# modelscope/dash-infer

Hardware: NVIDIA H100
Metric: decode tokens/sec/GPU Qwen2-7B int4-IQ b=1..64; HBM GB/s vs roofline (higher is better)
Workload: dtype bf16 activations x int4 weights (fp32 accumulate), none KV

## Files before the change

### dash-infer_b200/csrc/wq_gemm.cu

```cuda
#include <cstdio>
#include <cstdlib>
#include <cstring>
#include <map>
#include <mutex>
#include <new>

#include "b2_common.cuh"
#include "comm_shared.cuh"
#include "wq_gemm_shared.cuh"

namespace b2 {

constexpr int kWarps = 8;
constexpr int kThreads = kWarps * 32 + 32;
constexpr int kStageBytes = 8192;
static_assert(kBN == kWarps * 16, "one n16 tile per consumer warp");

struct GemmParams {
  const uint8_t* packed;
  const float2* sz;
  const __nv_bfloat16* A;
  int64_t lda;
  __nv_bfloat16* C;
  int64_t ldc;
// ... 736 lines not shown
    const __nv_bfloat16* sc = (pair && r >= 64) ? scales2 : scales;
    const __nv_bfloat16* zr = (pair && r >= 64) ? zeros2 : zeros;
    float2 v = make_float2(0.f, 0.f);
    if (n < N) {
      const __nv_bfloat16 sv = sc[(int64_t)gi * N + n], zv = zr[(int64_t)gi * N + n];
      v = fp16 ? make_float2(Ft<true>::to_f(sv), Ft<true>::to_f(zv) + zbias) : make_float2(Ft<false>::to_f(sv), Ft<false>::to_f(zv) + zbias);
    }
    dst[i] = v;
  }
}

}

using namespace b2;

struct Plan {
  bool valid = false;
  int S = 1, xt = 1, smem = 0, quanta = 1, nst_log2 = 2;
  bool cluster = false;
};

struct b2_gemm_wq {
  b2_gemm_wq_desc d;
  int Kp = 0, Np = 0, KT = 0, NG = 0, G = 1, group_tiles = 0;
  int group_k = 0;
  size_t tile_bytes = 0, packed_bytes = 0;
  void* packed = nullptr;
  bool own_packed = false;
  float2* sz = nullptr;
  bool own_sz = false;
  unsigned* counters = nullptr;
  Plan plans[2];
  int tc_S = 0;
  int tc_S2 = 0;
  bool pair = false;
  int device = 0;
};

typedef void (*gemm_kernel_t)(const GemmParams);

template <int WBITS, bool GROUPED, bool H>
static gemm_kernel_t pick_mt(int mt) {
  switch (mt) {
    case 1: return wq_gemm_kernel<WBITS, 1, GROUPED, H>;
    default: return wq_gemm_kernel<WBITS, 2, GROUPED, H>;
  }
}
template <bool H>
static gemm_kernel_t pick_kernel_ft(int wbits, bool grouped, int mt) {
  if (wbits == 4) return grouped ? pick_mt<4, true, H>(mt) : pick_mt<4, false, H>(mt);
  if (wbits == 8) return grouped ? pick_mt<8, true, H>(mt) : pick_mt<8, false, H>(mt);
  return pick_mt<16, false, H>(mt);
}
static gemm_kernel_t pick_kernel(int wbits, bool grouped, int mt, bool fp16) {
  return fp16 ? pick_kernel_ft<true>(wbits, grouped, mt) : pick_kernel_ft<false>(wbits, grouped, mt);
}
static int stage_bytes_of(int wbits) { return wbits == 16 ? WTraits<16>::STAGE_BYTES : kStageBytes; }
static int tile_bytes_of(int wbits) { return wbits == 4 ? WTraits<4>::TILE_BYTES : (wbits == 8 ? WTraits<8>::TILE_BYTES : WTraits<16>::TILE_BYTES); }

static int env_int(const char* name, int dflt) {
  const char* v = getenv(name);
  return v ? atoi(v) : dflt;
}

cudaError_t b2::raise_smem_limit(const void* kern, int smem) {
  static std::mutex mu;
  static std::map<const void*, int> limit;
// ... 209 lines not shown
int b2_gemm_wq_attach_packed(b2_gemm_wq_t h, const void* packed, const void* scales_f32, const void* zeros_f32) {
  (void)zeros_f32;
  if (!h || !packed) return B2_ERR_PARAM;
  if (h->own_packed && h->packed) cudaFree(h->packed);
  h->packed = const_cast<void*>(packed);
  h->own_packed = false;
  if (scales_f32) {
    if (h->own_sz && h->sz) cudaFree(h->sz);
    h->sz = (float2*)const_cast<void*>(scales_f32);
    h->own_sz = false;
  }
  return B2_OK;
}

static int mt_index_for(int M) { return M <= 8 ? 0 : 1; }

constexpr int kTcMinM = 17;

static bool use_tc(const b2_gemm_wq* h, int M) {
  if (h->group_k > 0) return true;
  return M >= kTcMinM && (h->group_tiles == 0 || h->d.wbits == 4);
}

static int make_tc_plan(b2_gemm_wq* h) {
  if (h->tc_S > 0) return B2_OK;
  const int ctas = env_int("B2_GEMM_TC_CTAS_PER_SM", 1);
  auto split_for = [&](int slots, int smax) {
    int S = slots / h->NG;
    if (S > h->KT / 4) S = h->KT / 4;
    if (S > smax) S = smax;
    return S < 1 ? 1 : S;
  };
  h->tc_S = split_for(ctas * sm_count(), env_int("B2_GEMM_TC_MAX_SPLIT", 6));
  h->tc_S2 = split_for(env_int("B2_GEMM_TC_DUAL_SLOTS", 2) * sm_count(), env_int("B2_GEMM_TC_MAX_SPLIT2", 8));
  return B2_OK;
}

static bool tc_dual(const b2_gemm_wq* h) {
  static const int on = env_int("B2_GEMM_TC_DUAL", 1);
  if (!on || h->d.wbits != 4) return false;
  return on >= 2 || h->NG >= 2 * sm_count();
}

size_t b2_gemm_wq_workspace_bytes(b2_gemm_wq_t h, int M) {
  if (!h || M <= 0) return 0;
  if (use_tc(h, M)) {
    if (make_tc_plan(h) != B2_OK) return 0;
    const int sm = h->tc_S > h->tc_S2 ? h->tc_S : h->tc_S2;
    return sm <= 1 ? 16 : (size_t)h->NG * sm * kTcMaxM * kBN * sizeof(float) + 16;
  }
  const int mc = M > kGemvMaxM ? kGemvMaxM : M;
  const int mti = mt_index_for(mc);
  if (make_plan(h, mti) != B2_OK) return 0;
  const Plan& pl = h->plans[mti];
  if (pl.S <= 1 || pl.cluster) return 16;
  return (size_t)h->NG * pl.S * (8 << mti) * (kBN + 1) * sizeof(float) + 16;
}

size_t b2_gemm_wq_algo_bytes(b2_gemm_wq_t h, int M) {
  if (!h) return 0;
  const b2_gemm_wq_desc& d = h->d;
  const size_t mul = h->pair ? 2 : 1;
  size_t w = mul * (size_t)d.K * d.N * d.wbits / 8;
  size_t prm = d.wbits == 16 ? 0 : mul * (size_t)2 * 2 * h->G * d.N;
  return w + prm + (size_t)2 * M * ((size_t)d.K + d.N);
}

int b2_gemm_wq_sumsq_parts(b2_gemm_wq_t h) { return h ? h->NG : 0; }

int b2_gemm_wq_run(b2_gemm_wq_t h, const void* A, int64_t lda, void* C, int64_t ldc, int M, const void* bias,
                   const void* residual, int activation, float alpha, void* workspace, size_t workspace_bytes,
                   void* stream_) {
  return b2_gemm_wq_run_fused(h, A, lda, C, ldc, M, bias, residual, activation, alpha, workspace, workspace_bytes, nullptr, stream_);
}

extern "C" const void* b2_comm_device_view(b2_comm_t c);

static int run_impl(b2_gemm_wq_t h, const void* A, int64_t lda, void* C, int64_t ldc, int M, const void* bias,
                    const void* residual, int activation, float alpha, void* workspace, size_t workspace_bytes,
                    const b2_gemm_fuse* fuse, const CommDev* comm, void* stream_);

int b2_gemm_wq_run_fused(b2_gemm_wq_t h, const void* A, int64_t lda, void* C, int64_t ldc, int M, const void* bias,
// ... 55 lines not shown
                    const b2_gemm_fuse* fuse, const CommDev* comm, void* stream_) {
  if (!h || !A || !C || M <= 0) return B2_ERR_PARAM;
  const bool norm_self = fuse && !fuse->norm_sumsq && fuse->norm_gamma;
  const bool fused = fuse && (fuse->norm_sumsq || fuse->sumsq_out || norm_self || fuse->xg_out);
  if (fused && use_tc(h, M) && !comm) {
    const bool cons = fuse->norm_sumsq != nullptr, prod = fuse->xg_out != nullptr;
    if (norm_self || (cons && fuse->norm_gamma) || (fuse->sumsq_out && !prod)) return B2_ERR_UNSUPPORTED;
    if (cons && (fuse->norm_parts <= 0 || fuse->norm_hidden <= 0)) return B2_ERR_PARAM;
    if (prod) {
      if (!fuse->sumsq_out || !fuse->gamma_out || h->pair || activation != B2_ACT_NONE) return B2_ERR_PARAM;
      if ((h->d.N & 3) || (ldc & 3) || (fuse->ldxg & 3) || (reinterpret_cast<uintptr_t>(C) & 7) ||
          (reinterpret_cast<uintptr_t>(fuse->xg_out) & 7) || (reinterpret_cast<uintptr_t>(fuse->gamma_out) & 7) ||
          (residual && (reinterpret_cast<uintptr_t>(residual) & 7)) || (bias && (reinterpret_cast<uintptr_t>(bias) & 7)))
        return B2_ERR_UNSUPPORTED;
    }
  } else {
    if (norm_self && (fuse->norm_hidden != h->d.K || comm)) return B2_ERR_PARAM;
    if (norm_self && (reinterpret_cast<uintptr_t>(fuse->norm_gamma) & 15)) return B2_ERR_UNSUPPORTED;
    if (fused && (M > 16 || (h->pair && fuse->sumsq_out) || fuse->xg_out)) return B2_ERR_UNSUPPORTED;
    if (fuse && fuse->norm_sumsq && (!fuse->norm_gamma || fuse->norm_parts <= 0 || fuse->norm_hidden <= 0)) return B2_ERR_PARAM;
  }
  if (!h->packed) return B2_ERR_RUNTIME;
  if (M > h->d.max_m) return B2_ERR_LIMIT;
  if (h->group_k > 0 && comm) return B2_ERR_UNSUPPORTED;
  if (h->pair != (activation == B2_ACT_SWIGLU)) return B2_ERR_PARAM;
  if (activation != B2_ACT_SWIGLU && (activation < 0 || activation > B2_ACT_SIGMOID)) return B2_ERR_PARAM;
  if (h->pair && (bias || residual)) return B2_ERR_UNSUPPORTED;
  if ((reinterpret_cast<uintptr_t>(A) & 15) || (lda % 8) != 0) return B2_ERR_UNSUPPORTED;
  if (workspace_bytes < b2_gemm_wq_workspace_bytes(h, M)) return B2_ERR_PARAM;
  cudaStream_t stream = (cudaStream_t)stream_;
  const bool grouped = h->group_tiles > 0;
  if (use_tc(h, M) && !comm) {
    if (int st = make_tc_plan(h)) return st;
    const bool dual = tc_dual(h);
    const int tcs = dual ? h->tc_S2 : h->tc_S;
    if (tcs > 1 && !workspace) return B2_ERR_PARAM;
    for (int m0 = 0; m0 < M; m0 += kTcMaxM) {
      TcLaunch a;
      a.dual = dual;
      a.fp16 = h->d.ft == B2_DT_F16;
      a.packed = (const uint8_t*)h->packed; a.sz = h->sz;
      a.A = (const __nv_bfloat16*)A + (int64_t)m0 * lda; a.lda = lda;
      a.C = (__nv_bfloat16*)C + (int64_t)m0 * ldc; a.ldc = ldc;
      a.bias = (const __nv_bfloat16*)bias;
      a.residual = residual ? (const __nv_bfloat16*)residual + (int64_t)m0 * ldc : nullptr;
      a.ws = (float*)workspace; a.counters = h->counters;
      a.M = (M - m0) > kTcMaxM ? kTcMaxM : (M - m0);
      a.N = h->d.N; a.K = h->d.K; a.Np = h->Np; a.KT = h->KT; a.NG = h->NG; a.S = tcs;
      a.act = activation; a.alpha = alpha;
      a.group_tiles = h->group_tiles;
      a.group_k = h->group_k; a.ngroups = h->G;
      if (fused) {
        a.norm_ld = M;
        if (fuse->norm_sumsq) {
          a.norm_sumsq = fuse->norm_sumsq + m0; a.norm_parts = fuse->norm_parts;
          a.norm_inv_hidden = 1.0f / (float)fuse->norm_hidden; a.norm_eps = fuse->norm_eps;
        }
        if (fuse->xg_out) {
          a.sumsq_out = fuse->sumsq_out + m0;
          a.xg_out = (__nv_bfloat16*)fuse->xg_out + (int64_t)m0 * fuse->ldxg;
          a.gamma_out = (const __nv_bfloat16*)fuse->gamma_out; a.ldxg = fuse->ldxg;
        }
      }
      cudaError_t e = tc_launch(h->d.wbits, a, stream);
      if (e != cudaSuccess) {
        set_last_error("wq_gemm_tc launch", e);
        return B2_ERR_CUDA;
      }
    }
    return B2_OK;
  }
  if (h->d.wbits == 16 && M <= kGemvMaxM && !fused && !comm && h->d.ft == B2_DT_BF16) {
// ... 66 lines not shown
```

### dash-infer_b200/csrc/wq_gemm_shared.cuh

```cuda
#pragma once
#include <cuda.h>

#include "b2_common.cuh"

namespace b2 {

constexpr int kBN = 128;
constexpr int kBK = 64;
constexpr uint32_t kMask4 = 0x00780078u;
constexpr uint32_t kMagic = 0x41804180u;
constexpr uint32_t kMagicHi = 0x43804380u;

__host__ __device__ __forceinline__ int tile_swz(int wbits, int c) {
  return wbits == 4 ? 4 * (c & 1) : (wbits == 8 ? 2 * (c & 3) : 2 * ((c >> 1) & 3));
}

struct TcLaunch {
  const uint8_t* packed;
  const float2* sz;
  const __nv_bfloat16* A;
  int64_t lda;
  __nv_bfloat16* C;
  int64_t ldc;
  const __nv_bfloat16* bias;
  const __nv_bfloat16* residual;
  float* ws;
  unsigned* counters;
  int M, N, K, Np, KT, NG, S;
  int act;
  float alpha;
  const float* a_scale = nullptr;
  const float* tile_sums = nullptr;
  int group_tiles = 0;
  int group_k = 0, ngroups = 1;
  bool fp16 = false;
  bool dual = false;
  const float* norm_sumsq = nullptr;
  int norm_parts = 0, norm_ld = 0;
  float norm_inv_hidden = 0.f, norm_eps = 0.f;
  float* sumsq_out = nullptr;
  __nv_bfloat16* xg_out = nullptr;
  const __nv_bfloat16* gamma_out = nullptr;
  int64_t ldxg = 0;
};
struct Gemv2Launch {
  const uint8_t* packed;
  const __nv_bfloat16* A;
  int64_t lda;
  __nv_bfloat16* C;
  int64_t ldc;
  const __nv_bfloat16* bias;
  const __nv_bfloat16* residual;
  int M, N, K, KT, NG;
  bool pair;
  int act;
  float alpha;
};
struct Gemv2Plan {
  int cb_log2, xt, nst_log2, mt, grid, smem;
};
bool gemv2_plan(const Gemv2Launch& a, Gemv2Plan* plan);
cudaError_t gemv2_launch(const Gemv2Launch& a, const Gemv2Plan& plan, cudaStream_t stream);

constexpr int kGemvMaxM = 16;
constexpr int kTcMaxM = 64;
int tc_smem_bytes(int wbits, bool dual);
cudaError_t tc_launch(int wbits, const TcLaunch& a, cudaStream_t stream);

cudaError_t raise_smem_limit(const void* kern, int smem);

typedef CUresult (*EncodeTiledFn)(CUtensorMap*, CUtensorMapDataType, cuuint32_t, void*, const cuuint64_t*, const cuuint64_t*,
                                  const cuuint32_t*, const cuuint32_t*, CUtensorMapInterleave, CUtensorMapSwizzle,
                                  CUtensorMapL2promotion, CUtensorMapFloatOOBfill);
EncodeTiledFn encode_tiled();

}
```

### dash-infer_b200/csrc/wq_gemm_tc.cu

```cuda
#include <cstdlib>

#include "b2_common.cuh"
#include "wq_gemm_shared.cuh"

namespace b2 {

constexpr int kTcThreads = 384;
constexpr int kTcNM = 64;
constexpr int kTcNSW = 6;
constexpr int kTcNSX = 3;
constexpr int kTcXTile = kTcNM * 128;

__device__ __forceinline__ void wg_fence() { asm volatile("wgmma.fence.sync.aligned;" ::: "memory"); }
__device__ __forceinline__ void wg_commit() { asm volatile("wgmma.commit_group.sync.aligned;" ::: "memory"); }
template <int N>
__device__ __forceinline__ void wg_wait() { asm volatile("wgmma.wait_group.sync.aligned %0;" ::"n"(N) : "memory"); }
__device__ __forceinline__ void wg_fence_acc(float (&d)[32]) {
#pragma unroll
  for (int i = 0; i < 32; ++i) asm volatile("" : "+f"(d[i])::"memory");
}
__device__ __forceinline__ uint64_t wg_desc(uint32_t saddr) {
  return (uint64_t)((saddr >> 4) & 0x3FFF) | ((uint64_t)1 << 16) | ((uint64_t)(1024 >> 4) << 32) | ((uint64_t)1 << 62);
}

#define B2_WG_D16 "{%0,%1,%2,%3,%4,%5,%6,%7,%8,%9,%10,%11,%12,%13,%14,%15}"
#define B2_WG_D32                                                                                                          \
  "{%0,%1,%2,%3,%4,%5,%6,%7,%8,%9,%10,%11,%12,%13,%14,%15,%16,%17,%18,%19,%20,%21,%22,%23,%24,%25,%26,%27,%28,%29,%30,%31}"
#define B2_WG_ACC16(d)                                                                                                       \
  "+f"(d[0]), "+f"(d[1]), "+f"(d[2]), "+f"(d[3]), "+f"(d[4]), "+f"(d[5]), "+f"(d[6]), "+f"(d[7]), "+f"(d[8]), "+f"(d[9]), \
      "+f"(d[10]), "+f"(d[11]), "+f"(d[12]), "+f"(d[13]), "+f"(d[14]), "+f"(d[15])
#define B2_WG_ACC32(d)                                                                                                       \
  B2_WG_ACC16(d), "+f"(d[16]), "+f"(d[17]), "+f"(d[18]), "+f"(d[19]), "+f"(d[20]), "+f"(d[21]), "+f"(d[22]), "+f"(d[23]), \
      "+f"(d[24]), "+f"(d[25]), "+f"(d[26]), "+f"(d[27]), "+f"(d[28]), "+f"(d[29]), "+f"(d[30]), "+f"(d[31])

template <int KIND>
__device__ __forceinline__ void wg_mma(float (&d)[32], const uint32_t (&a)[4], uint64_t desc, bool n32) {
  if (n32) {
    if (KIND == 0)
      asm volatile("{\n\t.reg .pred p;\n\tsetp.ne.b32 p, %21, 0;\n\t"
                   "wgmma.mma_async.sync.aligned.m64n32k16.f32.bf16.bf16 " B2_WG_D16 ", {%16,%17,%18,%19}, %20, p, 1, 1, 0;\n\t}"
                   : B2_WG_ACC16(d) : "r"(a[0]), "r"(a[1]), "r"(a[2]), "r"(a[3]), "l"(desc), "r"(1));
    else if (KIND == 1)
      asm volatile("{\n\t.reg .pred p;\n\tsetp.ne.b32 p, %21, 0;\n\t"
                   "wgmma.mma_async.sync.aligned.m64n32k16.f32.f16.f16 " B2_WG_D16 ", {%16,%17,%18,%19}, %20, p, 1, 1, 0;\n\t}"
                   : B2_WG_ACC16(d) : "r"(a[0]), "r"(a[1]), "r"(a[2]), "r"(a[3]), "l"(desc), "r"(1));
    else
      asm volatile("{\n\t.reg .pred p;\n\tsetp.ne.b32 p, %21, 0;\n\t"
                   "wgmma.mma_async.sync.aligned.m64n32k32.f32.e4m3.e4m3 " B2_WG_D16 ", {%16,%17,%18,%19}, %20, p, 1, 1;\n\t}"
                   : B2_WG_ACC16(d) : "r"(a[0]), "r"(a[1]), "r"(a[2]), "r"(a[3]), "l"(desc), "r"(1));
  } else {
    if (KIND == 0)
      asm volatile("{\n\t.reg .pred p;\n\tsetp.ne.b32 p, %37, 0;\n\t"
                   "wgmma.mma_async.sync.aligned.m64n64k16.f32.bf16.bf16 " B2_WG_D32 ", {%32,%33,%34,%35}, %36, p, 1, 1, 0;\n\t}"
                   : B2_WG_ACC32(d) : "r"(a[0]), "r"(a[1]), "r"(a[2]), "r"(a[3]), "l"(desc), "r"(1));
    else if (KIND == 1)
      asm volatile("{\n\t.reg .pred p;\n\tsetp.ne.b32 p, %37, 0;\n\t"
                   "wgmma.mma_async.sync.aligned.m64n64k16.f32.f16.f16 " B2_WG_D32 ", {%32,%33,%34,%35}, %36, p, 1, 1, 0;\n\t}"
                   : B2_WG_ACC32(d) : "r"(a[0]), "r"(a[1]), "r"(a[2]), "r"(a[3]), "l"(desc), "r"(1));
    else
      asm volatile("{\n\t.reg .pred p;\n\tsetp.ne.b32 p, %37, 0;\n\t"
                   "wgmma.mma_async.sync.aligned.m64n64k32.f32.e4m3.e4m3 " B2_WG_D32 ", {%32,%33,%34,%35}, %36, p, 1, 1;\n\t}"
                   : B2_WG_ACC32(d) : "r"(a[0]), "r"(a[1]), "r"(a[2]), "r"(a[3]), "l"(desc), "r"(1));
  }
}

__device__ __forceinline__ uint32_t tc_prmt(uint32_t a, uint32_t b, uint32_t sel) {
  uint32_t d;
  asm("prmt.b32 %0, %1, %2, %3;" : "=r"(d) : "r"(a), "r"(b), "r"(sel));
  return d;
}
// ... 11 lines not shown
  uint32_t r;
  asm("lop3.b32 %0, %1, %2, %3, 0xD8;" : "=r"(r) : "r"(lo), "r"(hi), "r"(m));
  return r;
}

struct TcParams {
  const uint8_t* packed;
  const float2* sz;
  const __nv_bfloat16* A;
  int64_t lda;
  __nv_bfloat16* C;
  int64_t ldc;
  const __nv_bfloat16* bias;
  const __nv_bfloat16* residual;
  float* ws;
  unsigned* counters;
  int M, N, K, Np, KT, NG, S;
  int act;
  float alpha;
  const float* a_scale;
  const float* tile_sums;
  const float* norm_sumsq;
  int norm_parts, norm_ld;
  float norm_inv_hidden, norm_eps;
  float* sumsq_out;
  __nv_bfloat16* xg_out;
  const __nv_bfloat16* gamma_out;
  int64_t ldxg;
  int nm;
  int group_tiles;
  int group_k, ngroups;
};

template <int WBITS, bool MULTI, bool A8 = false, bool GROUPED = false, bool DUAL = false, bool H = false>
__global__ void __launch_bounds__(kTcThreads, DUAL ? 2 : 1) wq_gemm_tc_kernel(const TcParams p, const __grid_constant__ CUtensorMap amap) {
  constexpr int TILE_BYTES = WBITS == 4 ? 4096 : (WBITS == 8 ? 8192 : 16384);
  constexpr int NCH = WBITS == 4 ? 2 : (WBITS == 8 ? 4 : 8);
  constexpr int NSW = WBITS == 16 ? 4 : kTcNSW;
  constexpr int TPS = WBITS == 4 ? (DUAL ? 2 : 4) : 2;
  constexpr int KIND = A8 ? 2 : (H ? 1 : 0);
  static_assert(!A8 || WBITS == 4, "fp8 activations: int4 weights only");
  static_assert(!DUAL || (WBITS == 4 && !A8), "two CTAs per SM: int4 weights, 16-bit activations");
  static_assert(!H || !A8, "fp8 activations come with bf16 outputs");
  using F = Ft<H>;
  static_assert(!GROUPED || (!A8 && WBITS != 16), "sub-channel weights: bf16 activations, int4 / int8");
  const int XTILE_LD = p.nm * 128;
  constexpr int XTPS = A8 ? TPS / 2 : TPS;
  constexpr int WSTAGE = TPS * TILE_BYTES;
  constexpr int XSTAGE = XTPS * kTcXTile;
  extern __shared__ uint8_t smem_raw[];
  uint8_t* smem = reinterpret_cast<uint8_t*>((reinterpret_cast<uintptr_t>(smem_raw) + 1023) & ~uintptr_t(1023));
  uint8_t* xring = smem;
  uint8_t* wring = xring + kTcNSX * XSTAGE;
  float* suma = reinterpret_cast<float*>(wring + NSW * WSTAGE);
  uint64_t* bars = reinterpret_cast<uint64_t*>(suma + kTcNM);
  uint64_t* wfull = bars;
  uint64_t* wfree = wfull + kTcNSW;
  uint64_t* afull = wfree + kTcNSW;
  uint64_t* xsum = afull + kTcNSX;
  uint64_t* xfree = xsum + kTcNSX;
  float* ascale = reinterpret_cast<float*>(bars) + 64;
  __shared__ int s_is_last;

  const int tid = threadIdx.x, warp = tid >> 5, lane = tid & 31;
  const int nunits = p.NG * p.S;

  if (tid == 0) {
    for (int i = 0; i < NSW; ++i) { mbar_init(&wfull[i], 1); mbar_init(&wfree[i], 8); }
    for (int i = 0; i < kTcNSX; ++i) { mbar_init(&afull[i], 1); mbar_init(&xsum[i], 2); mbar_init(&xfree[i], 8); }
    fence_mbar_init();
  }
  __syncthreads();
  pdl_launch_dependents();

  int w_pre = 0;
  const int my_units = !MULTI ? 1 : ((int)blockIdx.x < nunits) ? (nunits - (int)blockIdx.x + (int)gridDim.x - 1) / (int)gridDim.x : 0;
  for (int uit = 0; uit < my_units; ++uit) {
  const int unit = (int)blockIdx.x + uit * (int)gridDim.x;
  const int ng = unit / p.S;
  const int s = unit - ng * p.S;
  const int kt0 = (int)((int64_t)s * p.KT / p.S), kt1 = (int)((int64_t)(s + 1) * p.KT / p.S);
  const int nt = kt1 - kt0;
  const int nst = (nt + TPS - 1) / TPS;
  const int gbase = MULTI ? uit * nst : 0;
  if (warp == 8) {
    if (lane == 0) {
      auto issue = [&](int g, const uint8_t* src, uint32_t bytes) {
        const int slot = g % NSW;
        if (g >= NSW) mbar_wait_backoff(&wfree[slot], ((g / NSW) & 1) ^ 1);
        mbar_arrive_expect_tx(&wfull[slot], bytes);
        bulk_g2s(wring + slot * WSTAGE, src, bytes, &wfull[slot]);
      };
      const uint8_t* wsrc = p.packed + ((size_t)ng * p.KT + kt0) * TILE_BYTES;
      for (int st = w_pre; st < nst; ++st) issue(gbase + st, wsrc + (size_t)st * WSTAGE, min(TPS, nt - st * TPS) * TILE_BYTES);
      w_pre = 0;
      const int nu = unit + gridDim.x;
      if (MULTI && nu < nunits) {
        const int ng2 = nu / p.S, s2 = nu - ng2 * p.S;
        const int k0 = (int)((int64_t)s2 * p.KT / p.S), k1 = (int)((int64_t)(s2 + 1) * p.KT / p.S);
        const int nt2 = k1 - k0, nst2 = (nt2 + TPS - 1) / TPS;
        const uint8_t* wsrc2 = p.packed + ((size_t)ng2 * p.KT + k0) * TILE_BYTES;
        w_pre = min(NSW, nst2);
        for (int st = 0; st < w_pre; ++st)
          issue(gbase + nst + st, wsrc2 + (size_t)st * WSTAGE, min(TPS, nt2 - st * TPS) * TILE_BYTES);
      }
    }
  } else if (warp == 9) {
    if (lane == 0) {
      pdl_wait();
// ... 30 lines not shown
    }
    if (!A8 && p.norm_sumsq) {
      pdl_wait();
      float ss = 0.f;
      if (xt < p.M)
        for (int i = 0; i < p.norm_parts; ++i) ss += __ldcg(p.norm_sumsq + (size_t)i * p.norm_ld + xt);
      ascale[xt] = rsqrtf(ss * p.norm_inv_hidden + p.norm_eps);
    }
    for (int st = 0; st < nst; ++st) {
      const int g = gbase + st;
      const int slot = g % kTcNSX;
      mbar_wait(&afull[slot], (g / kTcNSX) & 1);
      const int tiles = (WBITS == 16 || A8 || GROUPED || xt >= p.nm) ? 0 : min(TPS, nt - st * TPS);
      for (int ti = 0; ti < tiles; ++ti) {
        const uint32_t rbase = smem_u32(xring + slot * XSTAGE + ti * kTcXTile) + xt * 128;
#pragma unroll
        for (int c = 0; c < 8; c += 2) {
          const uint4 v = lds128(rbase + ((c ^ (xt & 7)) << 4));
          const uint4 w = lds128(rbase + (((c + 1) ^ (xt & 7)) << 4));
          r0 += (F::lo(v.x) + F::hi(v.x)) + (F::lo(v.y) + F::hi(v.y));
          r1 += (F::lo(v.z) + F::hi(v.z)) + (F::lo(v.w) + F::hi(v.w));
          r2 += (F::lo(w.x) + F::hi(w.x)) + (F::lo(w.y) + F::hi(w.y));
          r3 += (F::lo(w.z) + F::hi(w.z)) + (F::lo(w.w) + F::hi(w.w));
        }
      }
      __syncwarp();
      if (lane == 0) mbar_arrive(&xsum[slot]);
    }
    suma[xt] = (r0 + r1) + (r2 + r3);
    asm volatile("bar.sync 3, 320;" ::: "memory");
  } else {
    const int wg = warp >> 2, g8 = lane >> 2, t4 = lane & 3;
    const int rr0 = wg * 64 + (warp & 3) * 16 + g8, rr1 = rr0 + 8;
    const bool n32 = p.nm == 32;
    const float2 sz0 = (WBITS == 16 || GROUPED) ? make_float2(1.f, 0.f) : p.sz[ng * kBN + rr0];
    const float2 sz1 = (WBITS == 16 || GROUPED) ? make_float2(1.f, 0.f) : p.sz[ng * kBN + rr1];
    const uint32_t wring_u = smem_u32(wring), xring_u = smem_u32(xring);
    uint32_t off0[NCH], off1[NCH];
#pragma unroll
    for (int c = 0; c < NCH; ++c) {
      off0[c] = c * 2048 + ((rr0 ^ tile_swz(WBITS, c)) << 4);
      off1[c] = c * 2048 + ((rr1 ^ tile_swz(WBITS, c)) << 4);
    }
    const uint32_t sh4 = 4 * t4, sh8 = 8 * (t4 & 1), qsh = 16 * (t4 & 1), msel = (t4 & 1) ? 0xFBEAu : 0xD9C8u;
    const int wa = t4 >> 1;
    auto word = [](const uint4& v, int j) { return j == 0 ? v.x : (j == 1 ? v.y : (j == 2 ? v.z : v.w)); };

    float d[32], dt[32];
#pragma unroll
    for (int i = 0; i < 32; ++i) d[i] = dt[i] = 0.f;
    int prev_xs = -1;
    for (int st = 0; st < nst; ++st) {
      const int g = gbase + st;
      const int slot = g % NSW, xs = g % kTcNSX;
      uint32_t gs2[TPS][2], gc2[TPS][2];
      if (GROUPED && p.group_k == 0) {
#pragma unroll
        for (int ti = 0; ti < TPS; ++ti) {
          const int kt = min(kt0 + st * TPS + ti, kt1 - 1);
          const float2 z0 = __ldg(p.sz + (size_t)(kt / p.group_tiles) * p.Np + ng * kBN + rr0);
          const float2 z1 = __ldg(p.sz + (size_t)(kt / p.group_tiles) * p.Np + ng * kBN + rr1);
          const float c0 = (F::kBias + 8.f - z0.y) * z0.x, c1 = (F::kBias + 8.f - z1.y) * z1.x;
          if (DUAL) {
            gs2[ti][0] = F::pack(z0.x, z1.x);
            gc2[ti][0] = F::pack(c0, c1);
          } else {
            gs2[ti][0] = F::pack(z0.x, z0.x); gs2[ti][1] = F::pack(z1.x, z1.x);
            gc2[ti][0] = F::pack(c0, c0); gc2[ti][1] = F::pack(c1, c1);
          }
        }
      }
      mbar_wait(&wfull[slot], (g / NSW) & 1);
      mbar_wait(&afull[xs], (g / kTcNSX) & 1);
      const int tiles = min(TPS, nt - st * TPS);
#pragma unroll
      for (int ti = 0; ti < TPS; ++ti) {
        if (ti < tiles) {
          const uint32_t wt = wring_u + slot * WSTAGE + ti * TILE_BYTES;
          if (A8) {
            const uint64_t bd = wg_desc(xring_u + xs * XSTAGE + (ti >> 1) * kTcXTile) + (uint64_t)(4 * (ti & 1));
            uint32_t a[2][4];
#pragma unroll
            for (int c = 0; c < 2; ++c) {
              const uint4 v0 = lds128(wt + off0[c]), v1 = lds128(wt + off1[c]);
              a[c][0] = nib4_to_e4m3(word(v0, wa), qsh, msel);
              a[c][1] = nib4_to_e4m3(word(v1, wa), qsh, msel);
              a[c][2] = nib4_to_e4m3(word(v0, 2 + wa), qsh, msel);
              a[c][3] = nib4_to_e4m3(word(v1, 2 + wa), qsh, msel);
            }
            wg_fence();
#pragma unroll
            for (int c = 0; c < 2; ++c) wg_mma<KIND>(dt, a[c], bd + (uint64_t)(2 * c), n32);
          } else {
            const uint64_t bd = wg_desc(xring_u + xs * XSTAGE + ti * kTcXTile);
            if (WBITS == 4) {
              uint32_t a[4][4];
#pragma unroll
              for (int c = 0; c < 2; ++c) {
                const uint4 v0 = lds128(wt + off0[c]), v1 = lds128(wt + off1[c]);
#pragma unroll
                for (int h = 0; h < 2; ++h) {
                  uint32_t* f = a[2 * c + h];
                  f[0] = lop3_and_or(__funnelshift_r(word(v0, 2 * h), word(v0, 2 * h), sh4), kMask4, F::kMagic);
                  f[1] = lop3_and_or(__funnelshift_r(word(v1, 2 * h), word(v1, 2 * h), sh4), kMask4, F::kMagic);
                  f[2] = lop3_and_or(__funnelshift_r(word(v0, 2 * h + 1), word(v0, 2 * h + 1), sh4), kMask4, F::kMagic);
                  f[3] = lop3_and_or(__funnelshift_r(word(v1, 2 * h + 1), word(v1, 2 * h + 1), sh4), kMask4, F::kMagic);
                  if (GROUPED) {
                    uint32_t sw[4], cw[4];
                    if (p.group_k > 0) {
#pragma unroll
                      for (int e = 0; e < 4; ++e) {
                        const int k0 = (kt0 + st * TPS + ti) * kBK + 32 * c + 8 * (2 * h + (e >> 1));
                        const float2 z = __ldg(p.sz + (size_t)min(k0 / p.group_k, p.ngroups - 1) * p.Np + ng * kBN + ((e & 1) ? rr1 : rr0));
                        sw[e] = F::pack(z.x, z.x);
                        const float cc = (F::kBias + 8.f - z.y) * z.x;
                        cw[e] = F::pack(cc, cc);
                      }
                    } else {
#pragma unroll
                      for (int e = 0; e < 4; ++e) {
                        if (DUAL) {
                          sw[e] = __byte_perm(gs2[ti][0], 0, (e & 1) ? 0x3232 : 0x1010);
                          cw[e] = __byte_perm(gc2[ti][0], 0, (e & 1) ? 0x3232 : 0x1010);
                        } else {
                          sw[e] = gs2[ti][e & 1]; cw[e] = gc2[ti][e & 1];
                        }
                      }
                    }
#pragma unroll
                    for (int e = 0; e < 4; ++e) {
                      uint32_t t2;
                      if (H) {
                        asm("add.rn.f16x2 %0, %1, %2;" : "=r"(t2) : "r"(f[e]), "r"(0xD840D840u));
                        asm("fma.rn.f16x2 %0, %1, %2, %3;" : "=r"(f[e]) : "r"(t2), "r"(sw[e]), "r"(cw[e]));
                      } else {
                        asm("add.rn.bf16x2 %0, %1, %2;" : "=r"(t2) : "r"(f[e]), "r"(0xC1C0C1C0u));
                        asm("fma.rn.bf16x2 %0, %1, %2, %3;" : "=r"(f[e]) : "r"(t2), "r"(sw[e]), "r"(cw[e]));
                      }
                    }
                  }
                }
                if (DUAL) {
                  wg_fence();
                  wg_mma<KIND>(d, a[2 * c], bd + (uint64_t)(4 * c), n32);
                  wg_mma<KIND>(d, a[2 * c + 1], bd + (uint64_t)(4 * c + 2), n32);
                  wg_commit();
                  wg_wait<1>();
                }
              }
              if (!DUAL) {
                wg_fence();
#pragma unroll
                for (int kk = 0; kk < 4; ++kk) wg_mma<KIND>(d, a[kk], bd + (uint64_t)(2 * kk), n32);
              }
            } else if (WBITS == 16) {
              uint32_t a[4][4];
#pragma unroll
              for (int kk = 0; kk < 4; ++kk) {
                a[kk][0] = lds32(wt + off0[2 * kk] + 4 * t4);
                a[kk][1] = lds32(wt + off1[2 * kk] + 4 * t4);
                a[kk][2] = lds32(wt + off0[2 * kk + 1] + 4 * t4);
                a[kk][3] = lds32(wt + off1[2 * kk + 1] + 4 * t4);
              }
              wg_fence();
#pragma unroll
              for (int kk = 0; kk < 4; ++kk) wg_mma<KIND>(d, a[kk], bd + (uint64_t)(2 * kk), n32);
            } else {
              uint32_t lo[4][4], hi[4][4];
#pragma unroll
              for (int c = 0; c < 4; ++c) {
                const uint4 v0 = lds128(wt + off0[c]), v1 = lds128(wt + off1[c]);
                const uint32_t w[4] = {word(v0, wa), word(v1, wa), word(v0, 2 + wa), word(v1, 2 + wa)};
#pragma unroll
                for (int e = 0; e < 4; ++e) {
                  lo[c][e] = lop3_and_or(__funnelshift_r(w[e], w[e], sh8), kMask4, F::kMagic);
                  hi[c][e] = lop3_and_or(__funnelshift_r(w[e], w[e], sh8 + 4), kMask4, F::kMagicHi);
                }
              }
              wg_fence();
#pragma unroll
              for (int c = 0; c < 4; ++c) {
                wg_mma<KIND>(d, lo[c], bd + (uint64_t)(2 * c), n32);
                wg_mma<KIND>(d, hi[c], bd + (uint64_t)(2 * c), n32);
              }
            }
          }
          if (!DUAL) {
            wg_commit();
            wg_wait<1>();
          }
          if (ti == 0 && prev_xs >= 0) {
            __syncwarp();
            if (lane == 0) mbar_arrive(&xfree[prev_xs]);
            prev_xs = -1;
          }
          if (A8 && ((ti & 1) || ti + 1 == tiles)) {
            wg_wait<0>();
            wg_fence_acc(dt);
#pragma unroll
            for (int i = 0; i < 32; ++i) { d[i] += dt[i]; dt[i] = 0.f; }
          }
        }
      }
      __syncwarp();
      if (lane == 0) mbar_arrive(&wfree[slot]);
      prev_xs = xs;
    }
    wg_wait<0>();
    wg_fence_acc(d);
    __syncwarp();
    if (prev_xs >= 0 && lane == 0) mbar_arrive(&xfree[prev_xs]);

    asm volatile("bar.sync 3, 320;" ::: "memory");
    float* fs = reinterpret_cast<float*>(xring);
#pragma unroll
    for (int j = 0; j < 8; ++j) {
      const int m = 8 * j + 2 * t4;
      float s0 = 1.f, s1 = 1.f;
      if (A8 || p.norm_sumsq) { s0 = ascale[m]; s1 = ascale[m + 1]; }
      const float zz0 = A8 ? sz0.y - 16.f : sz0.y, zz1 = A8 ? sz1.y - 16.f : sz1.y;
      const float sa0 = suma[m], sa1 = suma[m + 1];
      fs[m * kBN + rr0] = sz0.x * s0 * (d[4 * j + 0] - zz0 * sa0);
      fs[(m + 1) * kBN + rr0] = sz0.x * s1 * (d[4 * j + 1] - zz0 * sa1);
// ... 122 lines not shown
#pragma unroll 1
        for (int i = tid; i < p.M * (kBN / 2); i += T) {
          const int m = i >> 6, np = i & 63;
          const int nn = ng * kBN + np * 2;
          if (nn >= p.N) continue;
          float v0 = fs[m * kBN + np * 2] * p.alpha, v1 = fs[m * kBN + np * 2 + 1] * p.alpha;
          const bool has1 = (nn + 1) < p.N;
          if (p.bias) {
            v0 += F::to_f(p.bias[nn]);
            if (has1) v1 += F::to_f(p.bias[nn + 1]);
          }
          v0 = apply_act_rt(v0, p.act);
          v1 = apply_act_rt(v1, p.act);
          __nv_bfloat16* cp = p.C + (int64_t)m * p.ldc + nn;
          if (p.residual) {
            const __nv_bfloat16* rp = p.residual + (int64_t)m * p.ldc + nn;
            v0 += F::to_f(rp[0]);
            if (has1) v1 += F::to_f(rp[1]);
          }
          if (has1 && ((reinterpret_cast<uintptr_t>(cp) & 3) == 0)) {
            *reinterpret_cast<uint32_t*>(cp) = F::pack(v0, v1);
          } else {
            cp[0] = F::from_f(v0);
            if (has1) cp[1] = F::from_f(v1);
          }
        }
      }
    }
  }

  if (MULTI) asm volatile("fence.proxy.async.shared::cta;" ::: "memory");
  __syncthreads();
  }
}

int tc_smem_bytes(int wbits, bool dual) {
  const int tps = wbits == 4 ? (dual ? 2 : 4) : 2;
  const int wstage = tps * (wbits == 4 ? 4096 : (wbits == 8 ? 8192 : 16384));
  const int nsw = wbits == 16 ? 4 : kTcNSW;
  return 1024 + kTcNSX * tps * kTcXTile + nsw * wstage + kTcNM * 4 + 96 * 8 + 64;
}

EncodeTiledFn encode_tiled() {
  static EncodeTiledFn fn = nullptr;
  if (!fn) {
    void* p = nullptr;
    cudaDriverEntryPointQueryResult q;
    if (cudaGetDriverEntryPoint("cuTensorMapEncodeTiled", &p, cudaEnableDefault, &q) == cudaSuccess && q == cudaDriverEntryPointSuccess)
      fn = reinterpret_cast<EncodeTiledFn>(p);
  }
  return fn;
}

cudaError_t tc_launch(int wbits, const TcLaunch& a, cudaStream_t stream) {
  EncodeTiledFn enc = encode_tiled();
  if (!enc) return cudaErrorNotSupported;
  alignas(64) CUtensorMap amap;
  const bool a8 = a.a_scale != nullptr;
  const cuuint64_t gdim[2] = {(cuuint64_t)a.K, (cuuint64_t)a.M};
  const cuuint64_t gstride[1] = {(cuuint64_t)a.lda * (a8 ? 1 : 2)};
  static const int n32 = [] { const char* e = getenv("B2_GEMM_TC_N32"); return e ? atoi(e) : 1; }();
  const int nm = (n32 && a.M <= 32) ? 32 : kTcNM;
  const cuuint32_t box[2] = {(cuuint32_t)(a8 ? 2 * kBK : kBK), (cuuint32_t)nm};
  const cuuint32_t estr[2] = {1, 1};
  if (enc(&amap, a8 ? CU_TENSOR_MAP_DATA_TYPE_UINT8 : CU_TENSOR_MAP_DATA_TYPE_BFLOAT16, 2, const_cast<__nv_bfloat16*>(a.A), gdim, gstride, box, estr,
          CU_TENSOR_MAP_INTERLEAVE_NONE, CU_TENSOR_MAP_SWIZZLE_128B, CU_TENSOR_MAP_L2_PROMOTION_L2_128B,
          CU_TENSOR_MAP_FLOAT_OOB_FILL_NONE) != CUDA_SUCCESS)
    return cudaErrorInvalidValue;

  TcParams p;
  p.packed = a.packed; p.sz = a.sz; p.A = a.A; p.lda = a.lda; p.C = a.C; p.ldc = a.ldc; p.bias = a.bias; p.residual = a.residual;
  p.ws = a.ws; p.counters = a.counters; p.M = a.M; p.N = a.N; p.K = a.K; p.Np = a.Np; p.KT = a.KT; p.NG = a.NG; p.S = a.S;
  p.act = a.act; p.alpha = a.alpha;
  p.a_scale = a.a_scale; p.tile_sums = a.tile_sums;
  p.norm_sumsq = a.norm_sumsq; p.norm_parts = a.norm_parts; p.norm_ld = a.norm_ld; p.norm_inv_hidden = a.norm_inv_hidden;
  p.norm_eps = a.norm_eps; p.sumsq_out = a.sumsq_out; p.xg_out = a.xg_out; p.gamma_out = a.gamma_out; p.ldxg = a.ldxg;
  p.nm = nm; p.group_tiles = a.group_tiles; p.group_k = a.group_k; p.ngroups = a.ngroups;
  static const int persist = [] { const char* e = getenv("B2_GEMM_TC_PERSIST"); return e ? atoi(e) : 1; }();
  const int units = a.NG * a.S;
  const bool dual = a.dual && wbits == 4 && !a8;
  const int cap = (dual ? 2 : 1) * sm_count();
  const int grid = (persist && units > cap) ? cap : units;
  const bool multi = units > grid;
  const size_t smem = (size_t)tc_smem_bytes(wbits, dual);
  auto go = [&](auto kern) {
    const cudaError_t e = raise_smem_limit((const void*)kern, (int)smem);
    return e != cudaSuccess ? e : launch(kern, dim3(grid), dim3(kTcThreads), smem, stream, true, p, amap);
  };
  const bool g = a.group_tiles > 0 || a.group_k > 0, h = a.fp16;
  if (a8) {
    if (wbits != 4 || h) return cudaErrorNotSupported;
    return multi ? go(wq_gemm_tc_kernel<4, true, true>) : go(wq_gemm_tc_kernel<4, false, true>);
  }
  if (g && wbits != 4) return cudaErrorNotSupported;
  if (wbits == 4) {
    switch ((multi ? 8 : 0) | (g ? 4 : 0) | (dual ? 2 : 0) | (h ? 1 : 0)) {
      case 0: return go(wq_gemm_tc_kernel<4, false, false, false, false, false>);
      case 1: return go(wq_gemm_tc_kernel<4, false, false, false, false, true>);
      case 2: return go(wq_gemm_tc_kernel<4, false, false, false, true, false>);
      case 3: return go(wq_gemm_tc_kernel<4, false, false, false, true, true>);
      case 4: return go(wq_gemm_tc_kernel<4, false, false, true, false, false>);
      case 5: return go(wq_gemm_tc_kernel<4, false, false, true, false, true>);
      case 6: return go(wq_gemm_tc_kernel<4, false, false, true, true, false>);
      case 7: return go(wq_gemm_tc_kernel<4, false, false, true, true, true>);
      case 8: return go(wq_gemm_tc_kernel<4, true, false, false, false, false>);
      case 9: return go(wq_gemm_tc_kernel<4, true, false, false, false, true>);
      case 10: return go(wq_gemm_tc_kernel<4, true, false, false, true, false>);
      case 11: return go(wq_gemm_tc_kernel<4, true, false, false, true, true>);
      case 12: return go(wq_gemm_tc_kernel<4, true, false, true, false, false>);
      case 13: return go(wq_gemm_tc_kernel<4, true, false, true, false, true>);
      case 14: return go(wq_gemm_tc_kernel<4, true, false, true, true, false>);
      default: return go(wq_gemm_tc_kernel<4, true, false, true, true, true>);
    }
  }
  if (wbits == 16) {
    if (h) return multi ? go(wq_gemm_tc_kernel<16, true, false, false, false, true>) : go(wq_gemm_tc_kernel<16, false, false, false, false, true>);
    return multi ? go(wq_gemm_tc_kernel<16, true>) : go(wq_gemm_tc_kernel<16, false>);
  }
  if (h) return multi ? go(wq_gemm_tc_kernel<8, true, false, false, false, true>) : go(wq_gemm_tc_kernel<8, false, false, false, false, true>);
  return multi ? go(wq_gemm_tc_kernel<8, true>) : go(wq_gemm_tc_kernel<8, false>);
}

}
```

Measured before the change: 7145.

## Drop dual-CTA tensor-core GEMM path and specialize wgmma width at compile time

```diff
diff --git a/dash-infer_b200/csrc/wq_gemm.cu b/dash-infer_b200/csrc/wq_gemm.cu
--- a/dash-infer_b200/csrc/wq_gemm.cu
+++ b/dash-infer_b200/csrc/wq_gemm.cu
@@ -792,7 +792,6 @@
   unsigned* counters = nullptr;
   Plan plans[2];
   int tc_S = 0;
-  int tc_S2 = 0;
   bool pair = false;
   int device = 0;
 };
@@ -1068,22 +1067,14 @@
     return S < 1 ? 1 : S;
   };
   h->tc_S = split_for(ctas * sm_count(), env_int("B2_GEMM_TC_MAX_SPLIT", 6));
-  h->tc_S2 = split_for(env_int("B2_GEMM_TC_DUAL_SLOTS", 2) * sm_count(), env_int("B2_GEMM_TC_MAX_SPLIT2", 8));
   return B2_OK;
-}
-
-static bool tc_dual(const b2_gemm_wq* h) {
-  static const int on = env_int("B2_GEMM_TC_DUAL", 1);
-  if (!on || h->d.wbits != 4) return false;
-  return on >= 2 || h->NG >= 2 * sm_count();
 }
 
 size_t b2_gemm_wq_workspace_bytes(b2_gemm_wq_t h, int M) {
   if (!h || M <= 0) return 0;
   if (use_tc(h, M)) {
     if (make_tc_plan(h) != B2_OK) return 0;
-    const int sm = h->tc_S > h->tc_S2 ? h->tc_S : h->tc_S2;
-    return sm <= 1 ? 16 : (size_t)h->NG * sm * kTcMaxM * kBN * sizeof(float) + 16;
+    return h->tc_S <= 1 ? 16 : (size_t)h->NG * h->tc_S * kTcMaxM * kBN * sizeof(float) + 16;
   }
   const int mc = M > kGemvMaxM ? kGemvMaxM : M;
   const int mti = mt_index_for(mc);
@@ -1205,12 +1196,10 @@
   const bool grouped = h->group_tiles > 0;
   if (use_tc(h, M) && !comm) {
     if (int st = make_tc_plan(h)) return st;
-    const bool dual = tc_dual(h);
-    const int tcs = dual ? h->tc_S2 : h->tc_S;
+    const int tcs = h->tc_S;
     if (tcs > 1 && !workspace) return B2_ERR_PARAM;
     for (int m0 = 0; m0 < M; m0 += kTcMaxM) {
       TcLaunch a;
-      a.dual = dual;
       a.fp16 = h->d.ft == B2_DT_F16;
       a.packed = (const uint8_t*)h->packed; a.sz = h->sz;
       a.A = (const __nv_bfloat16*)A + (int64_t)m0 * lda; a.lda = lda;
diff --git a/dash-infer_b200/csrc/wq_gemm_shared.cuh b/dash-infer_b200/csrc/wq_gemm_shared.cuh
--- a/dash-infer_b200/csrc/wq_gemm_shared.cuh
+++ b/dash-infer_b200/csrc/wq_gemm_shared.cuh
@@ -34,7 +34,6 @@
   int group_tiles = 0;
   int group_k = 0, ngroups = 1;
   bool fp16 = false;
-  bool dual = false;
   const float* norm_sumsq = nullptr;
   int norm_parts = 0, norm_ld = 0;
   float norm_inv_hidden = 0.f, norm_eps = 0.f;
@@ -64,7 +63,7 @@
 
 constexpr int kGemvMaxM = 16;
 constexpr int kTcMaxM = 64;
-int tc_smem_bytes(int wbits, bool dual);
+int tc_smem_bytes(int wbits);
 cudaError_t tc_launch(int wbits, const TcLaunch& a, cudaStream_t stream);
 
 cudaError_t raise_smem_limit(const void* kern, int smem);
diff --git a/dash-infer_b200/csrc/wq_gemm_tc.cu b/dash-infer_b200/csrc/wq_gemm_tc.cu
--- a/dash-infer_b200/csrc/wq_gemm_tc.cu
+++ b/dash-infer_b200/csrc/wq_gemm_tc.cu
@@ -1,4 +1,5 @@
 #include <cstdlib>
+#include <type_traits>
 
 #include "b2_common.cuh"
 #include "wq_gemm_shared.cuh"
@@ -33,9 +34,9 @@
   B2_WG_ACC16(d), "+f"(d[16]), "+f"(d[17]), "+f"(d[18]), "+f"(d[19]), "+f"(d[20]), "+f"(d[21]), "+f"(d[22]), "+f"(d[23]), \
       "+f"(d[24]), "+f"(d[25]), "+f"(d[26]), "+f"(d[27]), "+f"(d[28]), "+f"(d[29]), "+f"(d[30]), "+f"(d[31])
 
-template <int KIND>
-__device__ __forceinline__ void wg_mma(float (&d)[32], const uint32_t (&a)[4], uint64_t desc, bool n32) {
-  if (n32) {
+template <int KIND, bool N32>
+__device__ __forceinline__ void wg_mma(float (&d)[32], const uint32_t (&a)[4], uint64_t desc) {
+  if constexpr (N32) {
     if (KIND == 0)
       asm volatile("{\n\t.reg .pred p;\n\tsetp.ne.b32 p, %21, 0;\n\t"
                    "wgmma.mma_async.sync.aligned.m64n32k16.f32.bf16.bf16 " B2_WG_D16 ", {%16,%17,%18,%19}, %20, p, 1, 1, 0;\n\t}"
@@ -113,15 +114,14 @@
   int group_k, ngroups;
 };
 
-template <int WBITS, bool MULTI, bool A8 = false, bool GROUPED = false, bool DUAL = false, bool H = false>
-__global__ void __launch_bounds__(kTcThreads, DUAL ? 2 : 1) wq_gemm_tc_kernel(const TcParams p, const __grid_constant__ CUtensorMap amap) {
+template <int WBITS, bool MULTI, bool A8 = false, bool GROUPED = false, bool H = false>
+__global__ void __launch_bounds__(kTcThreads, 1) wq_gemm_tc_kernel(const TcParams p, const __grid_constant__ CUtensorMap amap) {
   constexpr int TILE_BYTES = WBITS == 4 ? 4096 : (WBITS == 8 ? 8192 : 16384);
   constexpr int NCH = WBITS == 4 ? 2 : (WBITS == 8 ? 4 : 8);
   constexpr int NSW = WBITS == 16 ? 4 : kTcNSW;
-  constexpr int TPS = WBITS == 4 ? (DUAL ? 2 : 4) : 2;
+  constexpr int TPS = WBITS == 4 ? 4 : 2;
   constexpr int KIND = A8 ? 2 : (H ? 1 : 0);
   static_assert(!A8 || WBITS == 4, "fp8 activations: int4 weights only");
-  static_assert(!DUAL || (WBITS == 4 && !A8), "two CTAs per SM: int4 weights, 16-bit activations");
   static_assert(!H || !A8, "fp8 activations come with bf16 outputs");
   using F = Ft<H>;
   static_assert(!GROUPED || (!A8 && WBITS != 16), "sub-channel weights: bf16 activations, int4 / int8");
@@ -156,6 +156,8 @@
 
   int w_pre = 0;
   const int my_units = !MULTI ? 1 : ((int)blockIdx.x < nunits) ? (nunits - (int)blockIdx.x + (int)gridDim.x - 1) / (int)gridDim.x : 0;
+  auto body = [&](auto n32) {
+  constexpr bool N32 = decltype(n32)::value;
   for (int uit = 0; uit < my_units; ++uit) {
   const int unit = (int)blockIdx.x + uit * (int)gridDim.x;
   const int ng = unit / p.S;
@@ -252,7 +254,6 @@
   } else {
     const int wg = warp >> 2, g8 = lane >> 2, t4 = lane & 3;
     const int rr0 = wg * 64 + (warp & 3) * 16 + g8, rr1 = rr0 + 8;
-    const bool n32 = p.nm == 32;
     const float2 sz0 = (WBITS == 16 || GROUPED) ? make_float2(1.f, 0.f) : p.sz[ng * kBN + rr0];
     const float2 sz1 = (WBITS == 16 || GROUPED) ? make_float2(1.f, 0.f) : p.sz[ng * kBN + rr1];
     const uint32_t wring_u = smem_u32(wring), xring_u = smem_u32(xring);
@@ -281,13 +282,8 @@
           const float2 z0 = __ldg(p.sz + (size_t)(kt / p.group_tiles) * p.Np + ng * kBN + rr0);
           const float2 z1 = __ldg(p.sz + (size_t)(kt / p.group_tiles) * p.Np + ng * kBN + rr1);
           const float c0 = (F::kBias + 8.f - z0.y) * z0.x, c1 = (F::kBias + 8.f - z1.y) * z1.x;
-          if (DUAL) {
-            gs2[ti][0] = F::pack(z0.x, z1.x);
-            gc2[ti][0] = F::pack(c0, c1);
-          } else {
-            gs2[ti][0] = F::pack(z0.x, z0.x); gs2[ti][1] = F::pack(z1.x, z1.x);
-            gc2[ti][0] = F::pack(c0, c0); gc2[ti][1] = F::pack(c1, c1);
-          }
+          gs2[ti][0] = F::pack(z0.x, z0.x); gs2[ti][1] = F::pack(z1.x, z1.x);
+          gc2[ti][0] = F::pack(c0, c0); gc2[ti][1] = F::pack(c1, c1);
         }
       }
       mbar_wait(&wfull[slot], (g / NSW) & 1);
@@ -310,7 +306,7 @@
             }
             wg_fence();
 #pragma unroll
-            for (int c = 0; c < 2; ++c) wg_mma<KIND>(dt, a[c], bd + (uint64_t)(2 * c), n32);
+            for (int c = 0; c < 2; ++c) wg_mma<KIND, N32>(dt, a[c], bd + (uint64_t)(2 * c));
           } else {
             const uint64_t bd = wg_desc(xring_u + xs * XSTAGE + ti * kTcXTile);
             if (WBITS == 4) {
@@ -338,14 +334,7 @@
                       }
                     } else {
 #pragma unroll
-                      for (int e = 0; e < 4; ++e) {
-                        if (DUAL) {
-                          sw[e] = __byte_perm(gs2[ti][0], 0, (e & 1) ? 0x3232 : 0x1010);
-                          cw[e] = __byte_perm(gc2[ti][0], 0, (e & 1) ? 0x3232 : 0x1010);
-                        } else {
-                          sw[e] = gs2[ti][e & 1]; cw[e] = gc2[ti][e & 1];
-                        }
-                      }
+                      for (int e = 0; e < 4; ++e) { sw[e] = gs2[ti][e & 1]; cw[e] = gc2[ti][e & 1]; }
                     }
 #pragma unroll
                     for (int e = 0; e < 4; ++e) {
@@ -360,19 +349,10 @@
                     }
                   }
                 }
-                if (DUAL) {
-                  wg_fence();
-                  wg_mma<KIND>(d, a[2 * c], bd + (uint64_t)(4 * c), n32);
-                  wg_mma<KIND>(d, a[2 * c + 1], bd + (uint64_t)(4 * c + 2), n32);
-                  wg_commit();
-                  wg_wait<1>();
-                }
               }
-              if (!DUAL) {
-                wg_fence();
-#pragma unroll
-                for (int kk = 0; kk < 4; ++kk) wg_mma<KIND>(d, a[kk], bd + (uint64_t)(2 * kk), n32);
-              }
+              wg_fence();
+#pragma unroll
+              for (int kk = 0; kk < 4; ++kk) wg_mma<KIND, N32>(d, a[kk], bd + (uint64_t)(2 * kk));
             } else if (WBITS == 16) {
               uint32_t a[4][4];
 #pragma unroll
@@ -384,7 +364,7 @@
               }
               wg_fence();
 #pragma unroll
-              for (int kk = 0; kk < 4; ++kk) wg_mma<KIND>(d, a[kk], bd + (uint64_t)(2 * kk), n32);
+              for (int kk = 0; kk < 4; ++kk) wg_mma<KIND, N32>(d, a[kk], bd + (uint64_t)(2 * kk));
             } else {
               uint32_t lo[4][4], hi[4][4];
 #pragma unroll
@@ -400,15 +380,13 @@
               wg_fence();
 #pragma unroll
               for (int c = 0; c < 4; ++c) {
-                wg_mma<KIND>(d, lo[c], bd + (uint64_t)(2 * c), n32);
-                wg_mma<KIND>(d, hi[c], bd + (uint64_t)(2 * c), n32);
+                wg_mma<KIND, N32>(d, lo[c], bd + (uint64_t)(2 * c));
+                wg_mma<KIND, N32>(d, hi[c], bd + (uint64_t)(2 * c));
               }
             }
           }
-          if (!DUAL) {
-            wg_commit();
-            wg_wait<1>();
-          }
+          wg_commit();
+          wg_wait<1>();
           if (ti == 0 && prev_xs >= 0) {
             __syncwarp();
             if (lane == 0) mbar_arrive(&xfree[prev_xs]);
@@ -597,10 +575,15 @@
   if (MULTI) asm volatile("fence.proxy.async.shared::cta;" ::: "memory");
   __syncthreads();
   }
-}
-
-int tc_smem_bytes(int wbits, bool dual) {
-  const int tps = wbits == 4 ? (dual ? 2 : 4) : 2;
+  };
+  if (p.nm == 32)
+    body(std::true_type{});
+  else
+    body(std::false_type{});
+}
+
+int tc_smem_bytes(int wbits) {
+  const int tps = wbits == 4 ? 4 : 2;
   const int wstage = tps * (wbits == 4 ? 4096 : (wbits == 8 ? 8192 : 16384));
   const int nsw = wbits == 16 ? 4 : kTcNSW;
   return 1024 + kTcNSX * tps * kTcXTile + nsw * wstage + kTcNM * 4 + 96 * 8 + 64;
@@ -643,11 +626,10 @@
   p.nm = nm; p.group_tiles = a.group_tiles; p.group_k = a.group_k; p.ngroups = a.ngroups;
   static const int persist = [] { const char* e = getenv("B2_GEMM_TC_PERSIST"); return e ? atoi(e) : 1; }();
   const int units = a.NG * a.S;
-  const bool dual = a.dual && wbits == 4 && !a8;
-  const int cap = (dual ? 2 : 1) * sm_count();
+  const int cap = sm_count();
   const int grid = (persist && units > cap) ? cap : units;
   const bool multi = units > grid;
-  const size_t smem = (size_t)tc_smem_bytes(wbits, dual);
+  const size_t smem = (size_t)tc_smem_bytes(wbits);
   auto go = [&](auto kern) {
     const cudaError_t e = raise_smem_limit((const void*)kern, (int)smem);
     return e != cudaSuccess ? e : launch(kern, dim3(grid), dim3(kTcThreads), smem, stream, true, p, amap);
@@ -659,30 +641,22 @@
   }
   if (g && wbits != 4) return cudaErrorNotSupported;
   if (wbits == 4) {
-    switch ((multi ? 8 : 0) | (g ? 4 : 0) | (dual ? 2 : 0) | (h ? 1 : 0)) {
-      case 0: return go(wq_gemm_tc_kernel<4, false, false, false, false, false>);
-      case 1: return go(wq_gemm_tc_kernel<4, false, false, false, false, true>);
-      case 2: return go(wq_gemm_tc_kernel<4, false, false, false, true, false>);
-      case 3: return go(wq_gemm_tc_kernel<4, false, false, false, true, true>);
-      case 4: return go(wq_gemm_tc_kernel<4, false, false, true, false, false>);
-      case 5: return go(wq_gemm_tc_kernel<4, false, false, true, false, true>);
-      case 6: return go(wq_gemm_tc_kernel<4, false, false, true, true, false>);
-      case 7: return go(wq_gemm_tc_kernel<4, false, false, true, true, true>);
-      case 8: return go(wq_gemm_tc_kernel<4, true, false, false, false, false>);
-      case 9: return go(wq_gemm_tc_kernel<4, true, false, false, false, true>);
-      case 10: return go(wq_gemm_tc_kernel<4, true, false, false, true, false>);
-      case 11: return go(wq_gemm_tc_kernel<4, true, false, false, true, true>);
-      case 12: return go(wq_gemm_tc_kernel<4, true, false, true, false, false>);
-      case 13: return go(wq_gemm_tc_kernel<4, true, false, true, false, true>);
-      case 14: return go(wq_gemm_tc_kernel<4, true, false, true, true, false>);
-      default: return go(wq_gemm_tc_kernel<4, true, false, true, true, true>);
+    switch ((multi ? 4 : 0) | (g ? 2 : 0) | (h ? 1 : 0)) {
+      case 0: return go(wq_gemm_tc_kernel<4, false, false, false, false>);
+      case 1: return go(wq_gemm_tc_kernel<4, false, false, false, true>);
+      case 2: return go(wq_gemm_tc_kernel<4, false, false, true, false>);
+      case 3: return go(wq_gemm_tc_kernel<4, false, false, true, true>);
+      case 4: return go(wq_gemm_tc_kernel<4, true, false, false, false>);
+      case 5: return go(wq_gemm_tc_kernel<4, true, false, false, true>);
+      case 6: return go(wq_gemm_tc_kernel<4, true, false, true, false>);
+      default: return go(wq_gemm_tc_kernel<4, true, false, true, true>);
     }
   }
   if (wbits == 16) {
-    if (h) return multi ? go(wq_gemm_tc_kernel<16, true, false, false, false, true>) : go(wq_gemm_tc_kernel<16, false, false, false, false, true>);
+    if (h) return multi ? go(wq_gemm_tc_kernel<16, true, false, false, true>) : go(wq_gemm_tc_kernel<16, false, false, false, true>);
     return multi ? go(wq_gemm_tc_kernel<16, true>) : go(wq_gemm_tc_kernel<16, false>);
   }
-  if (h) return multi ? go(wq_gemm_tc_kernel<8, true, false, false, false, true>) : go(wq_gemm_tc_kernel<8, false, false, false, false, true>);
+  if (h) return multi ? go(wq_gemm_tc_kernel<8, true, false, false, true>) : go(wq_gemm_tc_kernel<8, false, false, false, true>);
   return multi ? go(wq_gemm_tc_kernel<8, true>) : go(wq_gemm_tc_kernel<8, false>);
 }
 
```

Measured after the change: 8008 (median of 6 runs). +12.1%, better.
